# will-rowe/hulk

Measured on AMD Instinct MI355X. Metric: reads/sec (150bp, k=21, sketch=512), higher is better.
Workload: dtype u64

## Files before the change

### hulk_amd/csrc/hulk_minimizer.hip

```cpp
#include "hulk_minhash.h"

#include <type_traits>

#include <math.h>
#include <stdlib.h>
#include <algorithm>

namespace hulk {
namespace {

__device__ __forceinline__ uint8_t nt4_of(unsigned c) {
    unsigned u = c | 0x20u;
    if (c < 4) return (uint8_t)c;
    if (u == 'a') return 0;
    if (u == 'c') return 1;
    if (u == 'g') return 2;
    if (u == 't' || u == 'u') return 3;
    return 4;
}

template <bool MH>
__global__ __launch_bounds__(256) void k_minimizer_bin(const uint8_t *__restrict__ bases,
                                                       const uint64_t *__restrict__ offsets,
                                                       uint64_t n_reads, MinimizerParams P,
// ... 117 lines not shown
            if (lane == 0) vm[j0 >> 6] = vmask;
        }
        wave_sync();

        uint64_t carry_m = 0; bool carry_emit = false;
        for (int32_t j0 = 0; j0 < npos; j0 += 64) {
            const int32_t j = j0 + lane;
            const int32_t i = j + k - 1;
            const uint64_t vmask = vm[j0 >> 6];
            const bool emit = (j < npos) && ((vmask >> lane) & 1ull) && (i >= w - 1);
            uint64_t m = X_NONE;
            if (emit) {
                int32_t lo = j - (wwin - 1); if (lo < 0) lo = 0;
                for (int32_t p = lo; p <= j; p++) { const uint64_t x = Xs[p]; m = x < m ? x : m; }
            }
            uint64_t pm = __shfl_up(m, 1);
            int pe = __shfl_up((int)emit, 1);
            if (lane == 0) { pm = carry_m; pe = (int)carry_emit; }
            carry_m = __shfl(m, 63); carry_emit = __shfl((int)emit, 63) != 0;
            const bool start = emit && !(pe && pm == m);
            bool isnew = false;
            if (dbg & 8u) { sink += (uint32_t)m; } else
            if (dbg & 4u) { isnew = start; } else
            if (start) {
                uint32_t slot = ((uint32_t)(m >> 8) ^ (uint32_t)(m >> 37)) & tabmask;
                for (;;) {
                    const unsigned long long old =
                        atomicCAS((unsigned long long *)&tab[slot], (unsigned long long)TAB_EMPTY,
                                  (unsigned long long)m);
                    if (old == TAB_EMPTY) { isnew = true; break; }
                    if (old == m) break;
                    slot = (slot + 1) & tabmask;
                }
            }
            const uint64_t nb = __ballot(isnew);
            if (nb) {
                const uint32_t rank = __builtin_amdgcn_mbcnt_hi((uint32_t)(nb >> 32),
                                          __builtin_amdgcn_mbcnt_lo((uint32_t)nb, 0u));
                if (isnew) { q[qn + rank] = m; qs[qn + rank] = hslot; }
                qn += (uint32_t)__popcll(nb);
                wave_sync();
            }
            if (qn >= 64) {
                const uint64_t x = q[lane];
                const uint32_t xs = qs[lane];
                const uint64_t keep = (lane + 64u < qn) ? q[lane + 64] : 0;
                const uint32_t keeps = (lane + 64u < qn) ? qs[lane + 64] : 0;
                if (MH) mh_feed_wave(M, x, true, mh_min);
                const int32_t bin = (dbg & 2u) ? (int32_t)((uint32_t)(x >> 20) & 0xffffu) : jump_hash(x, P.num_bins);
                if (dbg & 1u) sink += (uint32_t)bin; else
                atomicAdd(&hist[(size_t)xs * (size_t)P.num_bins + bin], 1u);
                wave_sync();
                q[lane] = keep; qs[lane] = keeps;
                wave_sync();
                qn -= 64; nmin += 64;
            }
        }
        for (uint32_t s = lane; s < tabn; s += 64) tab[s] = TAB_EMPTY;
        wave_sync();
    }
    if (qn) {
        if (MH) mh_feed_wave(M, (uint32_t)lane < qn ? q[lane] : ~0ull, (uint32_t)lane < qn, mh_min);
        if ((uint32_t)lane < qn)
            atomicAdd(&hist[(size_t)qs[lane] * (size_t)P.num_bins + jump_hash(q[lane], P.num_bins)], 1u);
        nmin += qn;
    }
    if (MH) mh_finish_wave(M, mh_min);
    __shared__ unsigned long long blk_nmin[4];
    if (lane == 0) blk_nmin[wid] = nmin;
    __syncthreads();
    if (threadIdx.x == 0) {
        unsigned long long t = 0;
        for (int x = 0; x < nw; x++) t += blk_nmin[x];
        if (t) atomicAdd(&min_slots[blockIdx.x], t);
        if (MH && t) atomicAdd(&M.fed[blockIdx.x & (MH_FED_SLOTS - 1)], t);
    }
    if (dbg && sink == 0xdeadbeefu) hist[0] = sink;
}


#ifndef HULK_FAST_TAB
#define HULK_FAST_TAB 128
#endif
#ifndef HULK_FAST_PAD
#define HULK_FAST_PAD 0
#endif
constexpr int FAST_TAB = HULK_FAST_TAB;
constexpr int FAST_PAD = HULK_FAST_PAD;
constexpr int FAST_CAND = 64;
constexpr int FAST_NCH = 3, FAST_NCH_PAIR = 5;
constexpr int FAST_STREAM = (64 * FAST_NCH + 4) * 4;
constexpr int FAST_STREAM_PAIR = (64 * FAST_NCH_PAIR + 4) * 4;
constexpr uint32_t TAB_EMPTY32 = 0xFFFFFFFFu;
constexpr int FAST_TAB_BYTES = 16 * FAST_TAB * 4;
static_assert(FAST_TAB > FAST_CAND, "the set must keep more slots than a read can have candidates (finite probe loops)");
static_assert((FAST_TAB & (FAST_TAB - 1)) == 0 && FAST_TAB % 16 == 0, "slot masks and the per-lane clear");
static_assert(2 * FAST_CAND <= 0x7fffffff, "candidate indices must not reach TAB_EMPTY32");

__device__ __forceinline__ uint32_t dpp_row_shr1(uint32_t v) {
    return (uint32_t)__builtin_amdgcn_update_dpp(0, (int)v, 0x111, 0xf, 0xf, true);
}
__device__ __forceinline__ uint64_t dpp_row_shr1_u64(uint64_t v) {
    return (uint64_t)dpp_row_shr1((uint32_t)v) | ((uint64_t)dpp_row_shr1((uint32_t)(v >> 32)) << 32);
}

__device__ __forceinline__ uint64_t mul_u32_u64(uint32_t a, uint32_t b) {
    uint64_t d, carry;
    asm("v_mad_u64_u32 %0, %1, %2, %3, 0" : "=v"(d), "=s"(carry) : "v"(a), "s"(b));
    return d;
}
__device__ __forceinline__ uint32_t mad_u24(uint32_t a, uint32_t b, uint32_t c) {
    uint32_t d;
    asm("v_mad_u32_u24 %0, %1, %2, %3" : "=v"(d) : "v"(a), "s"(b), "v"(c));
    return d;
}
template <uint32_t B> __device__ __forceinline__ uint64_t mul_u32_u64_inl(uint32_t a) {
    static_assert(B <= 64, "inline constants are 0..64");
    uint64_t d, carry;
    asm("v_mad_u64_u32 %0, %1, %2, %3, 0" : "=v"(d), "=s"(carry) : "v"(a), "n"(B));
    return d;
}
template <uint32_t B> __device__ __forceinline__ uint32_t mad_u24_inl(uint32_t a, uint32_t c) {
    static_assert(B <= 64, "inline constants are 0..64");
    uint32_t d;
    asm("v_mad_u32_u24 %0, %1, %2, %3" : "=v"(d) : "v"(a), "n"(B), "v"(c));
    return d;
}
template <bool FM> __device__ __forceinline__ uint64_t hash64_fm(uint64_t key, uint64_t mask) {
    if (!FM) return hash64(key, mask);
    key = (~key + (key << 21)) & mask;
    key = key ^ key >> 24;
    {
        const uint64_t p = mul_u32_u64((uint32_t)key, 265u);
        const uint32_t hi = mad_u24((uint32_t)(key >> 32), 265u, (uint32_t)(p >> 32));
        key = (((uint64_t)hi << 32) | (uint32_t)p) & mask;
    }
    key = key ^ key >> 14;
    {
        const uint64_t p = mul_u32_u64((uint32_t)key, 21u);
        const uint32_t hi = mad_u24((uint32_t)(key >> 32), 21u, (uint32_t)(p >> 32));
        key = (((uint64_t)hi << 32) | (uint32_t)p) & mask;
    }
    key = key ^ key >> 28;
    key = (key + (key << 31)) & mask;
    return key;
}

__device__ __forceinline__ uint64_t mad_u32_u64_m1(uint32_t a, uint32_t b) {
    uint64_t d, carry;
    asm("v_mad_u64_u32 %0, %1, %2, %3, -1" : "=v"(d), "=s"(carry) : "v"(a), "s"(b));
    return d;
}
template <int KC> __device__ __forceinline__ uint64_t hash64_pack_kc(uint64_t key, uint32_t span) {
    static_assert(KC >= 17 && KC <= 27, "upper dword of the k-mer must have 2..22 bits");
    constexpr uint32_t HM = (1u << (2 * KC - 32)) - 1u;
    uint32_t lo = (uint32_t)key, hi = (uint32_t)(key >> 32);
    uint64_t p;
    p = mad_u32_u64_m1(lo, 0x1FFFFFu);
    hi = mad_u24(hi, 0x1FFFFFu, (uint32_t)(p >> 32)) & HM; lo = (uint32_t)p;
    lo ^= __builtin_amdgcn_alignbit(hi, lo, 24);
    p = mul_u32_u64(lo, 265u);
    hi = mad_u24(hi, 265u, (uint32_t)(p >> 32)) & HM; lo = (uint32_t)p;
    lo ^= __builtin_amdgcn_alignbit(hi, lo, 14);
    if (2 * KC - 32 > 14) hi ^= hi >> 14;
    p = mul_u32_u64_inl<21u>(lo);
    hi = mad_u24_inl<21u>(hi, (uint32_t)(p >> 32)) & HM; lo = (uint32_t)p;
    lo ^= __builtin_amdgcn_alignbit(hi, lo, 28);
    p = mul_u32_u64(lo, 0x80000001u);
    hi = ((uint32_t)(p >> 32) + hi) & HM; lo = (uint32_t)p;
    const uint32_t xh = __builtin_amdgcn_alignbit(hi, lo, 24), xl = (lo << 8) | span;
    return ((uint64_t)xh << 32) | xl;
}

__device__ constexpr uint64_t low_bits64(int n) { return n >= 64 ? ~0ull : n <= 0 ? 0ull : (1ull << (n & 63)) - 1; }

template <int C> __device__ __forceinline__ uint32_t sub_c_if(uint32_t x, uint32_t one) {
    static_assert(C >= 1 && C <= 16, "-C must be an inline constant");
    uint32_t d;
    asm("v_mad_i32_i24 %0, %1, %2, %3" : "=v"(d) : "v"(one), "n"(-C), "v"(x));
    return d;
}
__device__ __forceinline__ uint32_t sub_small_if(uint32_t x, uint32_t one, int c) {
    switch (c) {
    case 1: return sub_c_if<1>(x, one);   case 2: return sub_c_if<2>(x, one);   case 3: return sub_c_if<3>(x, one);
    case 4: return sub_c_if<4>(x, one);   case 5: return sub_c_if<5>(x, one);   case 6: return sub_c_if<6>(x, one);
    case 7: return sub_c_if<7>(x, one);   case 8: return sub_c_if<8>(x, one);   case 9: return sub_c_if<9>(x, one);
    case 10: return sub_c_if<10>(x, one); case 11: return sub_c_if<11>(x, one); case 12: return sub_c_if<12>(x, one);
    case 13: return sub_c_if<13>(x, one); case 14: return sub_c_if<14>(x, one); case 15: return sub_c_if<15>(x, one);
    default: return x - one * (uint32_t)c;
    }
}

template <bool FM> __device__ __forceinline__ uint64_t umin64(uint64_t a, uint64_t b) {
    if (FM) {
        double d;
        asm("v_min_f64 %0, %1, %2" : "=v"(d) : "v"(__longlong_as_double((long long)a)), "v"(__longlong_as_double((long long)b)));
        return (uint64_t)__double_as_longlong(d);
    }
    return a < b ? a : b;
}

template <int WM, bool DBG, bool WEQ, int KC> constexpr int fast_blocks_per_cu() {
    return (WM == 9 && !DBG && WEQ && (KC == 21 || KC == 31)) ? 5 : 4;
}
template <int WM, bool FM, bool DBG, bool WEQ, int KC, bool PAIR>
__global__ __launch_bounds__(256, (fast_blocks_per_cu<WM, DBG, WEQ, KC>())) void k_minimizer_fast(const uint8_t *__restrict__ bases,
                                                        const uint64_t *__restrict__ offsets,
                                                        uint64_t n_reads, MinimizerParams P,
                                                        MinimizerList ml, DevState *st,
                                                        unsigned long long *__restrict__ min_slots) {
    extern __shared__ __align__(16) unsigned char smem[];

    constexpr bool KEY5 = !FM && WEQ && KC == 31;
    constexpr bool FMM = FM || KEY5;
    constexpr uint64_t XN = FMM ? 0x7FF0000000000000ull : X_NONE;
    const int lane = lane_id(), wid = __builtin_amdgcn_readfirstlane((int)(threadIdx.x >> 6));
    const int grp = threadIdx.x >> 4, gl = threadIdx.x & 15, gsh = lane & 48;
    const int32_t k = KC ? KC : (int32_t)P.k, w = WEQ ? WM : (int32_t)P.w;
    const uint64_t mask = (1ull << (2 * k)) - 1;
    const uint64_t shift = (uint64_t)(2 * (k - 1));
    constexpr int NCH = PAIR ? FAST_NCH_PAIR : FAST_NCH;
    constexpr int STW = (PAIR ? FAST_STREAM_PAIR : FAST_STREAM) / 4;
    constexpr uint32_t STCAP = 16u * 64u * NCH;
    constexpr int RPI = PAIR ? 2 : 4;
    constexpr bool DX = KC != 0 && WEQ && 2 * (KC + WM - 1) <= 64;
    constexpr bool HP = FM && WEQ && KC >= 17 && KC <= 27;
#ifdef HULK_ANALYSIS_NO_NV
    constexpr bool NV = false;
#else
    constexpr bool NV = (DX && HP && 2 * (KC + WM) <= 64) || (!DX && WM <= 9);
#endif
    const int half = PAIR ? (grp & 1) : 0;
    const int sub = PAIR ? ((grp & 3) >> 1) : (grp & 3);
    const int32_t posoff = half ? 16 * w - (w - 1) : 0;
    uint32_t *tab = (uint32_t *)(smem + FAST_PAD) + (size_t)(PAIR ? (grp & ~1) : grp) * FAST_TAB;
    uint32_t *pk32 = (uint32_t *)(smem + FAST_PAD + FAST_TAB_BYTES) + grp * 20;
    uint32_t *pkn32 = (uint32_t *)(smem + FAST_PAD + FAST_TAB_BYTES + 16 * 20 * 4) + grp * 20;
    uint32_t *code32 = (uint32_t *)(smem + FAST_PAD + FAST_TAB_BYTES + 2 * 16 * 20 * 4) + (size_t)wid * (2 * STW);
    uint32_t *flag32 = code32 + STW;
    uint64_t *cs = (uint64_t *)(smem + FAST_PAD + FAST_TAB_BYTES + 2 * 16 * 20 * 4 + 4 * 2 * 4 * STW) + (size_t)grp * FAST_CAND;
    const uint64_t *csp = PAIR ? cs - (size_t)half * FAST_CAND : cs;
    {
        uint32_t *own = (uint32_t *)(smem + FAST_PAD) + (size_t)grp * FAST_TAB;
#pragma unroll
        for (int x = 0; x < FAST_TAB / 16; x++) own[gl + 16 * x] = TAB_EMPTY32;
    }
    __syncthreads();

    const uint64_t region = (uint64_t)blockIdx.x * 4 + (uint64_t)wid;
    const uint64_t wave_first = region * FAST_READS_PER_WAVE;
    uint64_t *xl = ml.x + region * ml.rcap;
    uint8_t *sl8 = ml.slot + region * ml.rcap;
    uint32_t wcount = 0;
    uint32_t dmask = 0;
    const uint32_t dbg = DBG ? P.debug : 0u;
    uint32_t sink = 0;
    if (blockIdx.x == 0 && threadIdx.x == 0 && n_reads)
        atomicAdd(&st->total_len, (unsigned long long)(offsets[n_reads] - offsets[0]));

    const uint32_t nrd = wave_first < n_reads ? (uint32_t)((n_reads - wave_first < FAST_READS_PER_WAVE) ? n_reads - wave_first : FAST_READS_PER_WAVE) : 0u;
    uint64_t myoff = 0;
    if ((uint32_t)lane <= nrd && nrd) myoff = offsets[wave_first + (uint32_t)lane];
    const uint32_t nrd_s = __builtin_amdgcn_readfirstlane(nrd);
    const uint64_t span_lo = (uint64_t)__builtin_amdgcn_readfirstlane((uint32_t)myoff) | (uint64_t)__builtin_amdgcn_readfirstlane((uint32_t)(myoff >> 32)) << 32;
    const uint64_t span_hi = (uint64_t)__builtin_amdgcn_readlane((uint32_t)myoff, nrd_s) | (uint64_t)__builtin_amdgcn_readlane((uint32_t)(myoff >> 32), nrd_s) << 32;
    const uintptr_t raw_a0 = ((uintptr_t)bases + span_lo) & ~(uintptr_t)15;
    const uintptr_t raw_end = (uintptr_t)bases + span_hi;
    const bool bulk = nrd && (raw_end - raw_a0) <= (uintptr_t)STCAP;
    const uint32_t delta = (uint32_t)(((uintptr_t)bases + span_lo) - raw_a0);
    bool anymark = false;
    if (bulk) {
        const uintptr_t lim = (uintptr_t)bases + P.bases_bytes;
        uint4 v[NCH]; bool whole[NCH];
        const bool first_ok = raw_a0 < lim;
#pragma unroll
        for (int x = 0; x < NCH; x++) {
            const uintptr_t a = raw_a0 + 16u * (uint32_t)(lane + 64 * x);
            whole[x] = a < raw_end + 16 && a < lim;
            v[x] = first_ok ? *(const uint4 *)(whole[x] ? a : raw_a0) : make_uint4(0, 0, 0, 0);
        }
        const uint32_t endoff = (uint32_t)(raw_end - raw_a0);
        bool marked = false;
#pragma unroll
        for (int x = 0; x < NCH; x++) {
            const uint32_t d[4] = {v[x].x, v[x].y, v[x].z, v[x].w};
            uint32_t pack = 0, fpack = 0, bad = 0;
#pragma unroll
            for (int y = 0; y < 4; y++) {
                const uint32_t up = d[y] & 0xDFDFDFDFu;
                const uint32_t e = up >> 1;
                const uint32_t c = (e ^ (e >> 1)) & 0x03030303u;
                bad |= __builtin_amdgcn_perm(0u, 0x54474341u, c) ^ up;
                pack |= ((c * 0x01041040u) >> 24) << (8 * y);
            }
            if (!whole[x]) { pack = 0; bad = 0; }
            if (bad != 0) {
                const int32_t c0 = 16 * (lane + 64 * x);
                const int32_t lo = (int32_t)delta - c0, hi = (int32_t)endoff - c0;
#pragma unroll
                for (int y = 0; y < 4; y++) {
                    const uint32_t by = d[y], up = by & 0xDFDFDFDFu, e = up >> 1, c = (e ^ (e >> 1)) & 0x03030303u;
                    const int nl = lo - 4 * y, nh = hi - 4 * y;
                    const uint32_t ml = nl >= 4 ? ~0u : nl <= 0 ? 0u : (1u << (8 * nl)) - 1u;
                    const uint32_t mh = nh >= 4 ? ~0u : nh <= 0 ? 0u : (1u << (8 * nh)) - 1u;
                    const uint32_t mm = (__builtin_amdgcn_perm(0u, 0x54474341u, c) ^ up) & mh & ~ml;
                    const uint32_t nz = (((mm & 0x7F7F7F7Fu) + 0x7F7F7F7Fu) | mm) & 0x80808080u;
                    uint32_t hard4 = nz >> 7, soft4 = 0;
                    if (NV) {
                        const uint32_t tU = up ^ 0x55555555u, t3 = by & 0xFCFCFCFCu;
                        const uint32_t isU = ~(((tU & 0x7F7F7F7Fu) + 0x7F7F7F7Fu) | tU | 0x7F7F7F7Fu);
                        const uint32_t is03 = ~(((t3 & 0x7F7F7F7Fu) + 0x7F7F7F7Fu) | t3 | 0x7F7F7F7Fu);
                        hard4 = (nz & is03) >> 7;
                        soft4 = (nz & ~isU & ~is03) >> 7;
                    }
                    const uint32_t b4 = soft4 | (hard4 << 1);
                    const uint32_t fl = (b4 & 3u) | ((b4 >> 6) & 12u) | ((b4 >> 12) & 48u) | ((b4 >> 18) & 192u);
                    fpack |= fl << (8 * y);
                }
                pack &= ~((fpack & 0x55555555u) * 3u);
            }
            code32[lane + 64 * x] = pack;
            flag32[lane + 64 * x] = fpack;
            marked = marked || fpack != 0;
        }
        if (lane < 4) { code32[64 * NCH + lane] = 0u; flag32[64 * NCH + lane] = 0u; }
        anymark = __ballot(marked) != 0ull;
    }
    wave_sync();
// ... 60 lines not shown
        if (BULK) {
            cw = code32; fw = flag32;
            cb = a32 + (uint32_t)ap0; cb = cb < STCAP ? cb : STCAP;
            if (anymark) {
                Xn = win64(fw, ap0 ? cb - 1u : cb);
                if (ap0 == 0) Xn <<= 2;
                uint64_t seen;
                if (DX) {
                    constexpr int NBW = KC + WM - 1;
                    Xn &= low_bits64(2 * (NBW + 1));
                    seen = Xn;
                } else {
                    const uint32_t at = cb + (uint32_t)k;
                    nn = win32(fw, at < STCAP ? at : STCAP);
                    seen = Xn | nn;
                }
                const bool counts = act && !defer && p0 < nposg;
                sawN = counts && (seen & 0xAAAAAAAAAAAAAAAAull) != 0;
                softN = NV && counts && (seen & 0x5555555555555555ull) != 0;
                Xn &= 0x5555555555555555ull;
            }
        } else if (act && !defer) {
            const int32_t p = 16 * gl;
            uint32_t pack = 0, npack = 0;
            if (p < Lg) {
                const uint32_t ro = a32 + (uint32_t)posoff + (uint32_t)p;
                unsigned sh;
                uint32_t d[5];
                {
                    const uintptr_t addr = raw_a0 + ro;
                    const uintptr_t al = addr & ~(uintptr_t)3, end = (uintptr_t)bases + P.bases_bytes;
                    sh = (unsigned)(addr & 3) * 8;
#pragma unroll
                    for (int x = 0; x < 5; x++) d[x] = (al + 4 * x < end) ? *(const uint32_t *)(al + 4 * x) : 0u;
                }
                uint32_t bad = 0;
#pragma unroll
                for (int x = 0; x < 4; x++) {
                    const uint32_t by = __builtin_amdgcn_alignbit(d[x + 1], d[x], sh);
                    const uint32_t up = by & 0xDFDFDFDFu;
                    const uint32_t e = up >> 1;
                    const uint32_t c = (e ^ (e >> 1)) & 0x03030303u;
                    bad |= __builtin_amdgcn_perm(0u, 0x54474341u, c) ^ up;
                    pack |= ((c * 0x01041040u) >> 24) << (8 * x);
                }
                const bool lastread = Lg - p < 16 && lastwave && idx + 1 == nrd;
                if (bad != 0 || lastread) {
                    const int nv = lastread ? (int)(Lg - p) : 16;
                    uint32_t hard = 0;
#pragma unroll
                    for (int x = 0; x < 4; x++) {
                        const uint32_t by = __builtin_amdgcn_alignbit(d[x + 1], d[x], sh);
                        const uint32_t up = by & 0xDFDFDFDFu, e = up >> 1, c = (e ^ (e >> 1)) & 0x03030303u;
                        const int nb = nv - 4 * x;
                        const uint32_t m = nb >= 4 ? ~0u : nb <= 0 ? 0u : (1u << (8 * nb)) - 1u;
                        const uint32_t mm = (__builtin_amdgcn_perm(0u, 0x54474341u, c) ^ up) & m;
                        if (NV) {
                            const uint32_t nz = (((mm & 0x7F7F7F7Fu) + 0x7F7F7F7Fu) | mm) & 0x80808080u;
                            const uint32_t tU = up ^ 0x55555555u, t3 = by & 0xFCFCFCFCu;
                            const uint32_t isU = ~(((tU & 0x7F7F7F7Fu) + 0x7F7F7F7Fu) | tU | 0x7F7F7F7Fu);
                            const uint32_t is03 = ~(((t3 & 0x7F7F7F7Fu) + 0x7F7F7F7Fu) | t3 | 0x7F7F7F7Fu);
                            hard |= nz & is03;
                            const uint32_t b4 = (nz & ~isU & ~is03) >> 7;
                            const uint32_t fl = (b4 & 1u) | ((b4 >> 6) & 4u) | ((b4 >> 12) & 16u) | ((b4 >> 18) & 64u);
                            npack |= fl << (8 * x);
                        } else hard |= mm;
                    }
                    sawN = hard != 0;
                    softN = NV && npack != 0;
                    if (NV) pack &= ~(npack * 3u);
                }
            }
            pk32[gl] = pack;
            if (glq < 4) pk32[16 + gl] = 0;
            if (NV) { pkn32[gl] = npack; if (glq < 4) pkn32[16 + gl] = 0; }
        }
        const bool voting = !BULK || anymark;
        if (voting) {
            const uint32_t gN = PAIR ? (uint32_t)(__ballot(sawN) >> (lane & 32)) : (uint32_t)(__ballot(sawN) >> gsh) & 0xffffu;
            if (gN) defer = true;
        }
        const bool waveN = NV && voting && __ballot(softN && !defer) != 0ull;
        if (!BULK) wave_sync();
        if (dbg & 32u) { sink += cw[gl]; wave_sync(); return; }

        const bool mine = act && !defer && p0 < nposg;
        uint32_t validbits = 0;
        uint64_t X[WM];
#pragma unroll
        for (int t = 0; t < WM; t++) if (!WEQ || t >= w) X[t] = XN;
        {
            if (mine) validbits = (1u << (nposg - p0 < w ? nposg - p0 : w)) - 1u;
            const int32_t span0 = ap0 + k - 1 - w + 2;
            uint64_t f = 0, r = 0;
            uint32_t nb = 0;
            uint64_t Bb = 0, Cl = 0;
            uint64_t Hb = 0;
            if (NV && waveN && !BULK) {
                const uint32_t bo = 2u * (uint32_t)p0, nbo = p0 > 0 ? bo - 2u : 0u, d = nbo >> 5, o = nbo & 31u;
                const uint64_t lo = (uint64_t)pkn32[d] | ((uint64_t)pkn32[d + 1] << 32);
                Xn = o ? (lo >> o) | ((uint64_t)pkn32[d + 2] << (64 - o)) : lo;
                if (p0 == 0) {
                    Xn <<= 2;
                    if (PAIR && half) {
                        const uint32_t q = (uint32_t)(posoff - 1);
                        Xn |= (uint64_t)(((pkn32 - 20)[q >> 4] >> (2u * (q & 15u))) & 1u);
                    }
                }
            }
            if (DX) {
                constexpr int NBW = DX ? KC + WM - 1 : 1;
                uint64_t Wl = win64(cw, cb);
                Wl &= low_bits64(2 * NBW);
                const uint64_t rv = __brevll(Wl) >> (64 - 2 * NBW);
                Bb = ((rv >> 1) & 0x5555555555555555ull) | ((rv & 0x5555555555555555ull) << 1);
                Cl = ~Wl;
            } else {
                {
                    uint64_t W = win64(cw, cb);
                    W &= mask;
                    r = (~W) & mask;
                    if (NV && waveN) {
                        const uint64_t X0 = Xn & low_bits64(2 * k + 2);
                        W |= (X0 >> 4) & (mask >> 2);
                        r |= X0 & ((mask << 1) | 1ull);
                    }
                    const uint64_t rev = __brevll(W) >> (64 - 2 * k);
                    f = ((rev >> 1) & 0x5555555555555555ull) | ((rev & 0x5555555555555555ull) << 1);
                }
                {
                    uint32_t at = cb + (uint32_t)k;
                    if (BULK) at = at < STCAP ? at : STCAP;
                    nb = win32(cw, at);
                    if (NV && waveN && !BULK) nn = win32(fw, at);
                }
            }
            if (NV && DX && waveN) {
                constexpr int NBW = DX ? KC + WM - 1 : 1;
                Xn &= low_bits64(2 * (NBW + 1));
                const uint64_t Fn = (Xn >> 4) & low_bits64(2 * (NBW - 1));
                const uint64_t rv = __brevll(Fn) >> (64 - 2 * NBW);
                Hb = ((rv >> 1) & 0x5555555555555555ull) | ((rv & 0x5555555555555555ull) << 1);
            }
            uint32_t ap0_now = (uint32_t)ap0;
            if (KC != 0 && WEQ) asm volatile("" : "+v"(ap0_now));
            const bool first_block = ap0_now == 0u;
            const uint32_t fb1 = first_block ? 1u : 0u;
            auto phaseA = [&](auto nvx_tag) {
            constexpr bool NVX = decltype(nvx_tag)::value;
#pragma unroll
            for (int t = 0; t < WM; t++) {
                if (DX) {
                    constexpr int HB = 2 * KC - 32;
                    const int sf = 2 * (WM - 1 - t), sr = 2 * t;
                    const uint32_t bl = (uint32_t)Bb, cl = (uint32_t)Cl;
                    uint32_t bh = (uint32_t)(Bb >> 32), ch = (uint32_t)(Cl >> 32);
                    asm("" : "+v"(bh), "+v"(ch));
                    uint32_t fl = sf ? __builtin_amdgcn_alignbit(bh, bl, sf) : bl, fh = __builtin_amdgcn_ubfe(bh, sf, HB);
                    uint32_t rl = sr ? __builtin_amdgcn_alignbit(ch, cl, sr) : cl, rh = __builtin_amdgcn_ubfe(ch, sr, HB);
                    if (NVX) {
                        const uint32_t hl = (uint32_t)Hb, xl = (uint32_t)Xn;
                        uint32_t hh = (uint32_t)(Hb >> 32), xh = (uint32_t)(Xn >> 32);
                        asm("" : "+v"(hh), "+v"(xh));
                        fl |= (sf ? __builtin_amdgcn_alignbit(hh, hl, sf) : hl) & ~3u; fh |= __builtin_amdgcn_ubfe(hh, sf, HB);
                        rl |= sr ? __builtin_amdgcn_alignbit(xh, xl, sr) : xl; rh |= __builtin_amdgcn_ubfe(xh, sr, HB + 1);
                    }
                    f = ((uint64_t)fh << 32) | fl;
                    r = ((uint64_t)rh << 32) | rl;
                } else if (t) {
                    uint64_t c = nb & 3u; nb >>= 2;
                    if (NVX) { c |= (uint64_t)(nn & 1u) << 2; nn >>= 2; }
                    f = (f << 2 | c) & mask;
                    r = (r >> 2) | ((3ull ^ c) << shift);
                }
                if (t < w) {
                    const uint64_t canon = (NVX && k >= 31) ? (f < r ? f : r) : umin64<true>(f, r);
                    int32_t span;
                    if (KC != 0 && WEQ) span = k;
                    else { span = span0 + t; if (span >= k) span = k; }
                    uint64_t x;
                    if (HP && !(dbg & 16u)) x = hash64_pack_kc<HP ? KC : 21>(canon, (uint32_t)span);
                    else if (KEY5) x = (hash64(canon, mask) & 0x00FFFFFFFFFFFFFFull) << 5 | (uint64_t)(uint32_t)span;
                    else x = ((dbg & 16u) ? canon * 0x9E3779B97F4A7C15ull : hash64_fm<FM>(canon, mask)) << 8 | (uint64_t)(int64_t)span;
                    if (KC != 0 && WEQ && t < w - 1) x = (x & 0xffffffff00000000ull) | sub_small_if((uint32_t)x, fb1, w - 1 - t);
                    if ((NVX || !(k & 1)) && f == r) { x = XN; validbits &= ~(1u << t); }
                    X[t] = x;
                }
            }
            };
            if (NV && waveN) phaseA(std::true_type{}); else phaseA(std::false_type{});
        }
        if (dbg & 8u) {
#pragma unroll
            for (int t = 0; t < WM; t++) sink += (uint32_t)X[t];
            wave_sync();
            return;
        }

        uint32_t startbits = 0;
        {
            uint64_t hp[WM];
            {
                uint64_t h = XN;
#pragma unroll
                for (int t = WM - 1; t >= 0; t--) {
                    if (t < w) h = umin64<FMM>(X[t], h);
                    hp[t] = h;
                }
            }
            const uint64_t whole = dpp_row_shr1_u64(hp[0]);
            const uint64_t xnfix = glq == 0 ? XN : 0ull;
#pragma unroll
            for (int t = 0; t < WM - 1; t++) {
                const uint64_t v = dpp_row_shr1_u64(hp[t + 1]);
                hp[t] = FMM ? (v | (xnfix & 0xffffffff00000000ull)) : (v | xnfix);
            }
            hp[WM - 1] = XN;
            const uint32_t pv = dpp_row_shr1(validbits);
            uint32_t eqbits = 0;
            uint64_t g = XN, pm = whole;
#pragma unroll
            for (int t = 0; t < WM; t++) {
                g = umin64<FMM>(X[t], g);
                const uint64_t hpt = (t + 1 < w) ? hp[t] : XN;
                const uint64_t m = umin64<FMM>(hpt, g);
                if (t < w) { eqbits |= (m == pm) ? (1u << t) : 0u; pm = m; }
                X[t] = m;
            }
            uint32_t emitbits = validbits;
            {
                const int32_t t1 = (w - 1) - (k - 1) - ap0;
                if (t1 > 0) emitbits &= ~((1u << t1) - 1u);
                if (PAIR && halfq) { const int32_t t2 = (w - 1) - p0; if (t2 > 0) emitbits &= ~((1u << t2) - 1u); }
            }
            const uint32_t pe0 = (glq > 0 && ((pv >> (w - 1)) & 1u) && (ap0 - 1 + k - 1 >= w - 1) && !(halfq && p0 - 1 < w - 1)) ? 1u : 0u;
            startbits = emitbits & ~(((emitbits << 1) | pe0) & eqbits);
        }
        uint32_t total;
        {
            const uint32_t cnt = (uint32_t)__popc(startbits);
            uint32_t incl = cnt;
            incl += dpp_row_shr1(incl);
            incl += (uint32_t)__builtin_amdgcn_update_dpp(0, (int)incl, 0x112, 0xf, 0xf, true);
            incl += (uint32_t)__builtin_amdgcn_update_dpp(0, (int)incl, 0x114, 0xf, 0xf, true);
            incl += (uint32_t)__builtin_amdgcn_update_dpp(0, (int)incl, 0x118, 0xf, 0xf, true);
            total = (uint32_t)__shfl((int)incl, (lane & 48) | 15);
            bool ovf = total > (uint32_t)FAST_CAND;
            if (PAIR) ovf = ((uint32_t)(__ballot(ovf) >> (lane & 32))) != 0u;
            if (ovf) { defer = true; total = 0; }
            else {
                uint32_t at = incl - cnt;
#pragma unroll
                for (int t = 0; t < WM; t++)
                    if ((startbits >> t) & 1u) cs[at++] = X[t];
            }
        }
        {
            const uint64_t dbal = __ballot(act && defer && glq == 0 && halfq == 0);
            if (PAIR) dmask |= ((uint32_t)(dbal & 1u) | ((uint32_t)(dbal >> 32) & 1u) << 1) << (RPI * it);
            else dmask |= ((uint32_t)(dbal & 1u) | ((uint32_t)(dbal >> 16) & 1u) << 1 | ((uint32_t)(dbal >> 32) & 1u) << 2 |
                           ((uint32_t)(dbal >> 48) & 1u) << 3) << (RPI * it);
            if (act && defer) act = false;
        }
        wave_sync();

        uint32_t myslot[FAST_CAND / 16];
        uint32_t newmask = 0;
        constexpr uint32_t TABM = (PAIR ? 2 * FAST_TAB : FAST_TAB) - 1;
#pragma unroll
        for (int pr = 0; pr < FAST_CAND / 32; pr++) {
            const uint32_t c0 = (uint32_t)gl + 32u * (uint32_t)pr, c1 = c0 + 16u;
            myslot[2 * pr] = 0; myslot[2 * pr + 1] = 0;
            if (!__any((int)(c0 < total))) break;
            const bool a0 = c0 < total, a1 = c1 < total;
            uint64_t x0 = 0, x1 = 0;
            if (a0) x0 = cs[c0];
            if (a1) x1 = cs[c1];
            const uint64_t r0 = x0, r1 = x1;
            if (KEY5) { x0 = (x0 & ~31ull) << 3 | (x0 & 31ull); x1 = (x1 & ~31ull) << 3 | (x1 & 31ull); }
            uint32_t sl0 = ((uint32_t)(x0 >> 8) ^ (uint32_t)(x0 >> 37)) & TABM, sl1 = ((uint32_t)(x1 >> 8) ^ (uint32_t)(x1 >> 37)) & TABM;
            const uint32_t i0 = (PAIR ? (uint32_t)half * FAST_CAND : 0u) + c0, i1 = i0 + 16u;
            uint32_t o0 = TAB_EMPTY32, o1 = TAB_EMPTY32;
            if (!(dbg & 4u)) {
                if (a0) o0 = atomicCAS(&tab[sl0], TAB_EMPTY32, i0);
                if (a1) o1 = atomicCAS(&tab[sl1], TAB_EMPTY32, i1);
                while (a0 && o0 != TAB_EMPTY32 && csp[o0] != r0) {
                    sl0 = (sl0 + 1) & TABM;
                    o0 = atomicCAS(&tab[sl0], TAB_EMPTY32, i0);
                }
                while (a1 && o1 != TAB_EMPTY32 && csp[o1] != r1) {
                    sl1 = (sl1 + 1) & TABM;
                    o1 = atomicCAS(&tab[sl1], TAB_EMPTY32, i1);
                }
            }
            const bool new0 = a0 && o0 == TAB_EMPTY32, new1 = a1 && o1 == TAB_EMPTY32;
            myslot[2 * pr] = sl0; myslot[2 * pr + 1] = sl1;
            const uint64_t nb0 = __ballot(new0), nb1 = __ballot(new1);
            if (nb0 | nb1) {
                const uint32_t n0 = (uint32_t)__popcll(nb0);
                if (new0) {
                    const uint32_t rank = __builtin_amdgcn_mbcnt_hi((uint32_t)(nb0 >> 32), __builtin_amdgcn_mbcnt_lo((uint32_t)nb0, 0u));
                    newmask |= 1u << (2 * pr);
                    if (dbg & 1u) sink += (uint32_t)x0; else { xl[wcount + rank] = x0; sl8[wcount + rank] = (uint8_t)hslot; }
                }
                if (new1) {
                    const uint32_t rank = n0 + __builtin_amdgcn_mbcnt_hi((uint32_t)(nb1 >> 32), __builtin_amdgcn_mbcnt_lo((uint32_t)nb1, 0u));
                    newmask |= 2u << (2 * pr);
                    if (dbg & 1u) sink += (uint32_t)x1; else { xl[wcount + rank] = x1; sl8[wcount + rank] = (uint8_t)hslot; }
                }
                wcount += n0 + (uint32_t)__popcll(nb1);
            }
        }
        wave_sync();
#pragma unroll
        for (int rnd = 0; rnd < FAST_CAND / 16; rnd++)
            if ((newmask >> rnd) & 1u) tab[myslot[rnd]] = TAB_EMPTY32;
        wave_sync();
    };
    if (bulk) {
        for (int it = 0; it < FAST_READS_PER_WAVE / RPI && (uint32_t)(RPI * it) < nrd; it++) trip(std::true_type{}, it);
    } else if (!wide) {
        for (int it = 0; it < FAST_READS_PER_WAVE / RPI && (uint32_t)(RPI * it) < nrd; it++) trip(std::false_type{}, it);
    } else dmask = (1u << nrd_s) - 1u;
    if (lane == 0 && wave_first < n_reads) { ml.cnt[region] = wcount; ml.dmask[region] = dmask; }
    if (dbg && sink == 0xdeadbeefu) xl[0] = sink;
    __shared__ unsigned long long blk_nmin[4];
    if (lane == 0) blk_nmin[wid] = wcount;
    __syncthreads();
    if (threadIdx.x == 0) {
        const unsigned long long t = blk_nmin[0] + blk_nmin[1] + blk_nmin[2] + blk_nmin[3];
        if (t) atomicAdd(&min_slots[blockIdx.x & (MIN_SLOTS - 1)], t);
    }
}

#ifndef HULK_LONG_PPT
#define HULK_LONG_PPT 8
#endif
constexpr int LONG_PPT = HULK_LONG_PPT;
__global__ __launch_bounds__(256) void k_long_hash(const uint8_t *__restrict__ bases, const LongSeqDesc *__restrict__ desc,
                                                   MinimizerParams P, uint64_t *__restrict__ Xs_all,
                                                   uint8_t *__restrict__ valid_all) {
    __shared__ uint8_t lut[256];
    for (int t = threadIdx.x; t < 256; t += blockDim.x) lut[t] = nt4_of((unsigned)t);
    __syncthreads();
    const LongSeqDesc d = desc[blockIdx.y];
    const uint8_t *seq = bases + d.seq_off;
    uint64_t *Xs = Xs_all + d.xs_off;
    uint8_t *valid = valid_all + d.xs_off;
    const int64_t k = (int64_t)P.k, w = (int64_t)P.w;
    const uint64_t mask = (1ull << (2 * k)) - 1, shift = (uint64_t)(2 * (k - 1));
    const uint64_t npos = d.L - (uint64_t)k + 1;
    for (uint64_t j0 = ((uint64_t)blockIdx.x * blockDim.x + threadIdx.x) * LONG_PPT; j0 < npos;
         j0 += (uint64_t)gridDim.x * blockDim.x * LONG_PPT) {
        const uint64_t jend = j0 + LONG_PPT < npos ? j0 + LONG_PPT : npos;
        uint64_t f = 0, r = 0;
        for (int64_t p = j0 > 0 ? (int64_t)j0 - 1 : 0; p < (int64_t)jend + k - 1; p++) {
            const uint64_t c = lut[seq[p]];
            f = (f << 2 | c) & mask;
            r = (r >> 2) | ((3ull ^ c) << shift);
            const int64_t j = p - (k - 1);
            if (j < (int64_t)j0) continue;
            uint64_t X = X_NONE; uint8_t ok = 0;
            if (f != r) {
                const uint64_t canon = f > r ? r : f;
                int64_t span = p - w + 2;
                if (span >= k) span = k;
                X = hash64(canon, mask) << 8 | (uint64_t)(int64_t)(int32_t)span;
                ok = 1;
            }
            Xs[j] = X; valid[j] = ok;
        }
    }
}

__global__ __launch_bounds__(256) void k_long_emit(const LongSeqDesc *__restrict__ desc, const uint64_t *__restrict__ Xs_all,
                                                   const uint8_t *__restrict__ valid_all, MinimizerParams P,
                                                   uint64_t *__restrict__ table_all, uint32_t *__restrict__ hists,
                                                   unsigned long long *__restrict__ min_slots) {
    __shared__ unsigned red[4];
    constexpr unsigned QCAP = 2048;
    __shared__ uint64_t q[QCAP];
    __shared__ unsigned qn;
    if (threadIdx.x == 0) qn = 0;
    __syncthreads();
    const LongSeqDesc d = desc[blockIdx.y];
    const uint64_t *Xs = Xs_all + d.xs_off;
    const uint8_t *valid = valid_all + d.xs_off;
    uint64_t *table = table_all + d.tab_off;
    const uint64_t table_mask = d.tab_mask;
    uint32_t *hist = hists + (size_t)d.hslot * (size_t)P.num_bins;
    const int64_t k = (int64_t)P.k, w = (int64_t)P.w;
    const uint64_t wwin = (uint64_t)(w > 0 ? w : 1);
    const uint64_t npos = d.L - (uint64_t)k + 1;
    unsigned fresh = 0;
    for (uint64_t j0 = ((uint64_t)blockIdx.x * blockDim.x + threadIdx.x) * LONG_PPT; j0 < npos;
         j0 += (uint64_t)gridDim.x * blockDim.x * LONG_PPT) {
        const uint64_t jend = j0 + LONG_PPT < npos ? j0 + LONG_PPT : npos;
        uint64_t m = X_NONE, mprev = X_NONE;
// ... 130 lines not shown
                        const unsigned long long old = atomicCAS((unsigned long long *)&table[slot], (unsigned long long)TAB_EMPTY,
                                                                 (unsigned long long)m);
                        if (old == TAB_EMPTY) {
                            const unsigned at = atomicAdd(&qn, 1u);
                            if (at < QCAP) q[at] = m; else atomicAdd(&hist[jump_hash(m, P.num_bins)], 1u);
                            fresh++;
                            break;
                        }
                        if (old == m) break;
                        slot = (slot + 1) & table_mask;
                    }
                }
                prev_emit = emit; mprev = m;
            }
        }
        __syncthreads();
        {
#ifdef HULK_EXPERIMENTS
            if ((P.debug & LONG_TILE_LAG) && tid >= 64) {
                for (int i = 0; i < 10; i++) __builtin_amdgcn_s_sleep(127);
                __atomic_signal_fence(__ATOMIC_SEQ_CST);
            }
#endif
            const unsigned nq = qn < QCAP ? qn : QCAP;
            for (unsigned i = tid; i < nq; i += 256) atomicAdd(&hist[jump_hash(q[i], P.num_bins)], 1u);
        }
    }
    for (int off = 32; off; off >>= 1) fresh += __shfl_xor(fresh, off);
    if (lane_id() == 0) red[tid >> 6] = fresh;
    __syncthreads();
    if (tid == 0) {
        const unsigned t = red[0] + red[1] + red[2] + red[3];
        if (t) atomicAdd(&min_slots[(blockIdx.x + 131u * blockIdx.y) & (MIN_SLOTS - 1)], (unsigned long long)t);
    }
}

__global__ void k_fill_u64(uint64_t *p, uint64_t n, uint64_t v) {
    for (uint64_t i = (uint64_t)blockIdx.x * blockDim.x + threadIdx.x; i < n; i += (uint64_t)gridDim.x * blockDim.x) p[i] = v;
}

}

size_t minimizer_lds_per_wave(uint32_t xcap, uint32_t tab_size) {
    size_t words = (size_t)xcap + (xcap + 63) / 64 + tab_size + 128 + 64;
    size_t pk = ((size_t)xcap + 32 + 3) / 4 + 16;
    pk = (pk + 7) & ~(size_t)7;
    return words * 8 + 2 * pk;
}

size_t minimizer_lds_per_block(uint32_t xcap, uint32_t tab_size, int waves) {
    return 256 + (size_t)waves * minimizer_lds_per_wave(xcap, tab_size);
}

hipError_t launch_minimizer_bin(hipStream_t s, const uint8_t *d_bases, const uint64_t *d_offsets,
                                uint64_t n_reads, MinimizerParams P, int block_threads,
                                uint32_t *d_hist, DevState *d_state, unsigned long long *d_min_slots,
                                const uint32_t *d_read_list, const uint32_t *d_read_list_count,
                                uint32_t list_blocks, const MinHashState *mh) {
    if (n_reads == 0) return hipSuccess;
    const int waves = block_threads / 64;
    P.lds_per_wave = (uint32_t)minimizer_lds_per_wave(P.xcap, P.tab_size);
    const size_t lds = minimizer_lds_per_block(P.xcap, P.tab_size, waves);
    uint64_t blocks = (n_reads + (uint64_t)waves * 4 - 1) / ((uint64_t)waves * 4);
    if (blocks > MIN_SLOTS) blocks = MIN_SLOTS;
    if (blocks < 1) blocks = 1;
    if (d_read_list) blocks = list_blocks;
    const bool feed = mh && mh->mode;
    if (lds > 64 * 1024) {
        hipError_t e = hipFuncSetAttribute(feed ? (const void *)k_minimizer_bin<true> : (const void *)k_minimizer_bin<false>,
                                           hipFuncAttributeMaxDynamicSharedMemorySize, (int)lds);
        if (e != hipSuccess) return e;
    }
    prof_mark(s, "k_minimizer_bin");
    if (feed)
        hipLaunchKernelGGL(k_minimizer_bin<true>, dim3((unsigned)blocks), dim3(block_threads), lds, s, d_bases,
                           d_offsets, n_reads, P, d_hist, d_state, d_min_slots, d_read_list, d_read_list_count, *mh);
    else
        hipLaunchKernelGGL(k_minimizer_bin<false>, dim3((unsigned)blocks), dim3(block_threads), lds, s, d_bases,
                           d_offsets, n_reads, P, d_hist, d_state, d_min_slots, d_read_list, d_read_list_count, MinHashState{});
    return hipGetLastError();
}

constexpr size_t fast_lds_bytes(bool pair) {
    return FAST_PAD + (size_t)FAST_TAB_BYTES + 2 * 16 * 20 * 4 + 4 * 2 * (size_t)(pair ? FAST_STREAM_PAIR : FAST_STREAM) + 16 * (size_t)FAST_CAND * 8;
}
constexpr size_t FAST_LDS_GRANULE = 1280, FAST_LDS_STATIC = 32, CU_LDS_BYTES = 160 * 1024;
constexpr size_t fast_lds_alloc(bool pair) { return (fast_lds_bytes(pair) + FAST_LDS_STATIC + FAST_LDS_GRANULE - 1) / FAST_LDS_GRANULE * FAST_LDS_GRANULE; }
#if HULK_FAST_PAD == 0 && HULK_FAST_TAB == 128
static_assert(fast_blocks_per_cu<9, false, true, 21>() == 5 && fast_blocks_per_cu<9, false, true, 31>() == 5, "the default instances are built for 5 workgroups per CU");
static_assert(6 * fast_lds_alloc(false) <= CU_LDS_BYTES, "k_minimizer_fast: the LDS no longer admits 6 workgroups per CU (its registers are budgeted for 5)");
static_assert(5 * fast_lds_alloc(true) <= CU_LDS_BYTES, "k_minimizer_fast (PAIR): the LDS no longer admits the 5 workgroups per CU its registers are budgeted for");
#endif
size_t minimizer_fast_lds(uint32_t, bool pair) { return fast_lds_bytes(pair); }

hipError_t launch_minimizer_fast(hipStream_t s, const uint8_t *d_bases, const uint64_t *d_offsets,
                                 uint64_t n_reads, MinimizerParams P, const MinimizerList &ml,
                                 DevState *d_state, unsigned long long *d_min_slots) {
    if (n_reads == 0) return hipSuccess;
    const bool pair = P.pair != 0;
    size_t lds = minimizer_fast_lds(P.w, pair);
    {
        static const char *e = HULK_EXP_ENV("HULK_K1_LDS_TOTAL");
        static const size_t want = e ? (size_t)atol(e) : 0;
        if (want > lds) {
            static bool once = false;
            if (!once && want > 65536) { once = true; (void)hipFuncSetAttribute((const void *)k_minimizer_fast<9, false, false, true, 31, false>, hipFuncAttributeMaxDynamicSharedMemorySize, (int)want); }
            lds = want;
        }
    }
    const uint64_t blocks = (n_reads + 4 * FAST_READS_PER_WAVE - 1) / (4 * FAST_READS_PER_WAVE);
    const dim3 g((unsigned)blocks), b(256);
    static const bool no_fmin = HULK_EXP_ENV("HULK_NO_FMIN") != nullptr;
    const bool fm = P.k <= 27 && !no_fmin;
    prof_mark(s, "k_minimizer_fast");
#define HULK_LAUNCH_FAST3(WM, FMv, DBGv, WEQv, KCv, PAIRv)                                                           \
    hipLaunchKernelGGL((k_minimizer_fast<WM, FMv, DBGv, WEQv, KCv, PAIRv>), g, b, lds, s, d_bases, d_offsets, n_reads, \
                       P, ml, d_state, d_min_slots)
#define HULK_LAUNCH_FAST2(WM, FMv, DBGv, WEQv, KCv)                                                                  \
    do { if (pair) HULK_LAUNCH_FAST3(WM, FMv, DBGv, WEQv, KCv, true); else HULK_LAUNCH_FAST3(WM, FMv, DBGv, WEQv, KCv, false); } while (0)
#define HULK_LAUNCH_FAST(WM)                                                                                         \
    do {                                                                                                             \
        const bool weq = P.w == WM;                                                                                  \
        if (P.debug) HULK_LAUNCH_FAST2(WM, false, true, false, 0);                                                   \
        else if (fm && weq && P.k == 21) HULK_LAUNCH_FAST2(WM, true, false, true, 21);    \
        else if (!fm && weq && P.k == 31) HULK_LAUNCH_FAST2(WM, false, false, true, 31);           \
        else if (fm && weq) HULK_LAUNCH_FAST2(WM, true, false, true, 0);                                             \
        else if (fm) HULK_LAUNCH_FAST2(WM, true, false, false, 0);                                                   \
        else if (weq) HULK_LAUNCH_FAST2(WM, false, false, true, 0);                                                  \
        else HULK_LAUNCH_FAST2(WM, false, false, false, 0);                                                          \
    } while (0)
    if (P.w <= 4) HULK_LAUNCH_FAST(4);
    else if (P.w <= 9) HULK_LAUNCH_FAST(9);
    else HULK_LAUNCH_FAST(16);
#undef HULK_LAUNCH_FAST3
#undef HULK_LAUNCH_FAST2
#undef HULK_LAUNCH_FAST
    return hipGetLastError();
}

uint32_t minimizer_list_rcap(uint32_t w, bool pair) {
    static const uint32_t pad = [] { const char *e = HULK_EXP_ENV("HULK_RCAP_PAD"); return e ? (uint32_t)atol(e) : 64u; }();
    const uint32_t by_pos = FAST_READS_PER_WAVE * (pair ? 2u * 16u * w - (w - 1u) : 16u * w);
    const uint32_t by_cand = FAST_READS_PER_WAVE * (uint32_t)FAST_CAND * (pair ? 2u : 1u);
    return by_pos < by_cand + pad ? by_pos : by_cand + pad;
}

hipError_t launch_long_group(hipStream_t s, const uint8_t *d_bases, const LongSeqDesc *d_desc, uint32_t n_seqs,
                             uint64_t max_npos, MinimizerParams P, uint64_t *d_xs, uint8_t *d_valid, uint64_t *d_table,
                             uint64_t table_total, uint32_t *d_hists, unsigned long long *d_min_slots) {
    prof_mark(s, "k_fill_u64");
    hipLaunchKernelGGL(k_fill_u64, dim3(4096), dim3(256), 0, s, d_table, table_total, TAB_EMPTY);
    if (d_xs && d_valid) {
        uint64_t bx = (max_npos + 256 * LONG_PPT - 1) / (256 * LONG_PPT);
        const uint64_t cap = std::max<uint64_t>(1, 131072 / n_seqs);
        if (bx > cap) bx = cap;
        if (bx > 8192) bx = 8192;
        prof_mark(s, "k_long_hash");
        hipLaunchKernelGGL(k_long_hash, dim3((unsigned)bx, n_seqs), dim3(256), 0, s, d_bases, d_desc, P, d_xs, d_valid);
        prof_mark(s, "k_long_emit");
        hipLaunchKernelGGL(k_long_emit, dim3((unsigned)bx, n_seqs), dim3(256), 0, s, d_desc, d_xs, d_valid, P, d_table,
                           d_hists, d_min_slots);
        return hipGetLastError();
    }
    const uint64_t H = (((uint64_t)(P.w ? P.w : 1) + 7) & ~7ull), TP = (uint64_t)LONG_TILE - H;
    uint64_t bx = (max_npos + TP - 1) / TP;
    const uint64_t cap = std::max<uint64_t>(1, 262144 / n_seqs);
    if (bx > cap) bx = cap;
    if (bx > 65535) bx = 65535;
    if (const char *e = HULK_EXP_ENV("HULK_LONG_TILE_GRID")) { const long n = atol(e); if (n > 0 && bx > (uint64_t)n) bx = (uint64_t)n; }
    if (HULK_EXP_ENV("HULK_LONG_TILE_LAG")) P.debug |= LONG_TILE_LAG;
    prof_mark(s, "k_long_tile");
    hipLaunchKernelGGL(k_long_tile, dim3((unsigned)bx, n_seqs), dim3(256), 0, s, d_bases, d_desc, P, d_table, d_hists, d_min_slots);
    return hipGetLastError();
}

}
```

Before: 2.164 billion.

## Shrink single-read LDS footprint to fit seven workgroups per CU on headline path

Drops the per-group candidate cap from 64 to 48 for single-end reads. It also removes the separate pk32/pkn32 staging buffers by aliasing them into the per-wave code/flag streams, so the single-end LDS allocation shrinks. The headline instance (w=9, k=21, single-end) gets launch bounds of 7 workgroups per CU, and the bit offset is taken from a pinned register cb. The aim is higher occupancy. The risks are register spills under the tighter budget and more reads overflowing the smaller candidate set and being deferred to a slower path.

```diff
diff --git a/hulk_amd/csrc/hulk_minimizer.hip b/hulk_amd/csrc/hulk_minimizer.hip
--- a/hulk_amd/csrc/hulk_minimizer.hip
+++ b/hulk_amd/csrc/hulk_minimizer.hip
@@ -223,20 +223,26 @@
 #ifndef HULK_FAST_TAB
 #define HULK_FAST_TAB 128
 #endif
+#ifndef HULK_FAST_TAB_SINGLE
+#define HULK_FAST_TAB_SINGLE 128
+#endif
 #ifndef HULK_FAST_PAD
 #define HULK_FAST_PAD 0
 #endif
-constexpr int FAST_TAB = HULK_FAST_TAB;
 constexpr int FAST_PAD = HULK_FAST_PAD;
-constexpr int FAST_CAND = 64;
+constexpr int fast_tab(bool pair) { return pair ? HULK_FAST_TAB : HULK_FAST_TAB_SINGLE; }
+constexpr int fast_cand(bool pair) { return pair ? 64 : 48; }
 constexpr int FAST_NCH = 3, FAST_NCH_PAIR = 5;
 constexpr int FAST_STREAM = (64 * FAST_NCH + 4) * 4;
 constexpr int FAST_STREAM_PAIR = (64 * FAST_NCH_PAIR + 4) * 4;
 constexpr uint32_t TAB_EMPTY32 = 0xFFFFFFFFu;
-constexpr int FAST_TAB_BYTES = 16 * FAST_TAB * 4;
-static_assert(FAST_TAB > FAST_CAND, "the set must keep more slots than a read can have candidates (finite probe loops)");
-static_assert((FAST_TAB & (FAST_TAB - 1)) == 0 && FAST_TAB % 16 == 0, "slot masks and the per-lane clear");
-static_assert(2 * FAST_CAND <= 0x7fffffff, "candidate indices must not reach TAB_EMPTY32");
+constexpr int fast_tab_bytes(bool pair) { return 16 * fast_tab(pair) * 4; }
+static_assert(fast_tab(false) > fast_cand(false) && fast_tab(true) > fast_cand(true),
+              "the set must keep more slots than a read can have candidates (finite probe loops)");
+static_assert((fast_tab(false) & (fast_tab(false) - 1)) == 0 && fast_tab(false) % 16 == 0 &&
+              (fast_tab(true) & (fast_tab(true) - 1)) == 0 && fast_tab(true) % 16 == 0, "slot masks and the per-lane clear");
+static_assert(fast_cand(false) % 16 == 0 && fast_cand(true) % 16 == 0, "candidates are taken 16 per round (one per lane of a group)");
+static_assert(2 * fast_cand(true) <= 0x7fffffff, "candidate indices must not reach TAB_EMPTY32");
 
 __device__ __forceinline__ uint32_t dpp_row_shr1(uint32_t v) {
     return (uint32_t)__builtin_amdgcn_update_dpp(0, (int)v, 0x111, 0xf, 0xf, true);
@@ -341,11 +347,15 @@
     return a < b ? a : b;
 }
 
-template <int WM, bool DBG, bool WEQ, int KC> constexpr int fast_blocks_per_cu() {
+#ifndef HULK_FAST_HEADLINE_BLOCKS
+#define HULK_FAST_HEADLINE_BLOCKS 7
+#endif
+template <int WM, bool DBG, bool WEQ, int KC, bool PAIR> constexpr int fast_blocks_per_cu() {
+    if (WM == 9 && !DBG && WEQ && KC == 21 && !PAIR) return HULK_FAST_HEADLINE_BLOCKS;
     return (WM == 9 && !DBG && WEQ && (KC == 21 || KC == 31)) ? 5 : 4;
 }
 template <int WM, bool FM, bool DBG, bool WEQ, int KC, bool PAIR>
-__global__ __launch_bounds__(256, (fast_blocks_per_cu<WM, DBG, WEQ, KC>())) void k_minimizer_fast(const uint8_t *__restrict__ bases,
+__global__ __launch_bounds__(256, (fast_blocks_per_cu<WM, DBG, WEQ, KC, PAIR>())) void k_minimizer_fast(const uint8_t *__restrict__ bases,
                                                         const uint64_t *__restrict__ offsets,
                                                         uint64_t n_reads, MinimizerParams P,
                                                         MinimizerList ml, DevState *st,
@@ -371,20 +381,22 @@
 #else
     constexpr bool NV = (DX && HP && 2 * (KC + WM) <= 64) || (!DX && WM <= 9);
 #endif
+    constexpr int TABN = fast_tab(PAIR), CAND = fast_cand(PAIR), TAB_BYTES = fast_tab_bytes(PAIR);
     const int half = PAIR ? (grp & 1) : 0;
     const int sub = PAIR ? ((grp & 3) >> 1) : (grp & 3);
     const int32_t posoff = half ? 16 * w - (w - 1) : 0;
-    uint32_t *tab = (uint32_t *)(smem + FAST_PAD) + (size_t)(PAIR ? (grp & ~1) : grp) * FAST_TAB;
-    uint32_t *pk32 = (uint32_t *)(smem + FAST_PAD + FAST_TAB_BYTES) + grp * 20;
-    uint32_t *pkn32 = (uint32_t *)(smem + FAST_PAD + FAST_TAB_BYTES + 16 * 20 * 4) + grp * 20;
-    uint32_t *code32 = (uint32_t *)(smem + FAST_PAD + FAST_TAB_BYTES + 2 * 16 * 20 * 4) + (size_t)wid * (2 * STW);
+    uint32_t *tab = (uint32_t *)(smem + FAST_PAD) + (size_t)(PAIR ? (grp & ~1) : grp) * TABN;
+    uint32_t *code32 = (uint32_t *)(smem + FAST_PAD + TAB_BYTES) + (size_t)wid * (2 * STW);
     uint32_t *flag32 = code32 + STW;
-    uint64_t *cs = (uint64_t *)(smem + FAST_PAD + FAST_TAB_BYTES + 2 * 16 * 20 * 4 + 4 * 2 * 4 * STW) + (size_t)grp * FAST_CAND;
-    const uint64_t *csp = PAIR ? cs - (size_t)half * FAST_CAND : cs;
+    uint32_t *pk32 = code32 + (grp & 3) * 20;
+    uint32_t *pkn32 = flag32 + (grp & 3) * 20;
+    static_assert(4 * 20 <= STW, "the per-trip staging of a wave's four groups fits in each of its streams");
+    uint64_t *cs = (uint64_t *)(smem + FAST_PAD + TAB_BYTES + 4 * 2 * 4 * STW) + (size_t)grp * CAND;
+    const uint64_t *csp = PAIR ? cs - (size_t)half * CAND : cs;
     {
-        uint32_t *own = (uint32_t *)(smem + FAST_PAD) + (size_t)grp * FAST_TAB;
-#pragma unroll
-        for (int x = 0; x < FAST_TAB / 16; x++) own[gl + 16 * x] = TAB_EMPTY32;
+        uint32_t *own = (uint32_t *)(smem + FAST_PAD) + (size_t)grp * TABN;
+#pragma unroll
+        for (int x = 0; x < TABN / 16; x++) own[gl + 16 * x] = TAB_EMPTY32;
     }
     __syncthreads();
 
@@ -611,6 +623,7 @@
         }
         const bool waveN = NV && voting && __ballot(softN && !defer) != 0ull;
         if (!BULK) wave_sync();
+        if (!BULK && KC != 0 && WEQ) asm volatile("" : "+v"(cb));
         if (dbg & 32u) { sink += cw[gl]; wave_sync(); return; }
 
         const bool mine = act && !defer && p0 < nposg;
@@ -626,7 +639,7 @@
             uint64_t Bb = 0, Cl = 0;
             uint64_t Hb = 0;
             if (NV && waveN && !BULK) {
-                const uint32_t bo = 2u * (uint32_t)p0, nbo = p0 > 0 ? bo - 2u : 0u, d = nbo >> 5, o = nbo & 31u;
+                const uint32_t bo = 2u * cb, nbo = p0 > 0 ? bo - 2u : 0u, d = nbo >> 5, o = nbo & 31u;
                 const uint64_t lo = (uint64_t)pkn32[d] | ((uint64_t)pkn32[d + 1] << 32);
                 Xn = o ? (lo >> o) | ((uint64_t)pkn32[d + 2] << (64 - o)) : lo;
                 if (p0 == 0) {
@@ -774,7 +787,7 @@
             incl += (uint32_t)__builtin_amdgcn_update_dpp(0, (int)incl, 0x114, 0xf, 0xf, true);
             incl += (uint32_t)__builtin_amdgcn_update_dpp(0, (int)incl, 0x118, 0xf, 0xf, true);
             total = (uint32_t)__shfl((int)incl, (lane & 48) | 15);
-            bool ovf = total > (uint32_t)FAST_CAND;
+            bool ovf = total > (uint32_t)CAND;
             if (PAIR) ovf = ((uint32_t)(__ballot(ovf) >> (lane & 32))) != 0u;
             if (ovf) { defer = true; total = 0; }
             else {
@@ -793,22 +806,24 @@
         }
         wave_sync();
 
-        uint32_t myslot[FAST_CAND / 16];
+        constexpr int NRND = CAND / 16;
+        uint32_t myslot[NRND];
         uint32_t newmask = 0;
-        constexpr uint32_t TABM = (PAIR ? 2 * FAST_TAB : FAST_TAB) - 1;
-#pragma unroll
-        for (int pr = 0; pr < FAST_CAND / 32; pr++) {
+        constexpr uint32_t TABM = (PAIR ? 2 * TABN : TABN) - 1;
+#pragma unroll
+        for (int pr = 0; pr < (NRND + 1) / 2; pr++) {
+            const bool two = 2 * pr + 1 < NRND;
             const uint32_t c0 = (uint32_t)gl + 32u * (uint32_t)pr, c1 = c0 + 16u;
-            myslot[2 * pr] = 0; myslot[2 * pr + 1] = 0;
+            myslot[2 * pr] = 0; if (two) myslot[2 * pr + 1] = 0;
             if (!__any((int)(c0 < total))) break;
-            const bool a0 = c0 < total, a1 = c1 < total;
+            const bool a0 = c0 < total, a1 = two && c1 < total;
             uint64_t x0 = 0, x1 = 0;
             if (a0) x0 = cs[c0];
             if (a1) x1 = cs[c1];
             const uint64_t r0 = x0, r1 = x1;
             if (KEY5) { x0 = (x0 & ~31ull) << 3 | (x0 & 31ull); x1 = (x1 & ~31ull) << 3 | (x1 & 31ull); }
             uint32_t sl0 = ((uint32_t)(x0 >> 8) ^ (uint32_t)(x0 >> 37)) & TABM, sl1 = ((uint32_t)(x1 >> 8) ^ (uint32_t)(x1 >> 37)) & TABM;
-            const uint32_t i0 = (PAIR ? (uint32_t)half * FAST_CAND : 0u) + c0, i1 = i0 + 16u;
+            const uint32_t i0 = (PAIR ? (uint32_t)half * CAND : 0u) + c0, i1 = i0 + 16u;
             uint32_t o0 = TAB_EMPTY32, o1 = TAB_EMPTY32;
             if (!(dbg & 4u)) {
                 if (a0) o0 = atomicCAS(&tab[sl0], TAB_EMPTY32, i0);
@@ -823,7 +838,7 @@
                 }
             }
             const bool new0 = a0 && o0 == TAB_EMPTY32, new1 = a1 && o1 == TAB_EMPTY32;
-            myslot[2 * pr] = sl0; myslot[2 * pr + 1] = sl1;
+            myslot[2 * pr] = sl0; if (two) myslot[2 * pr + 1] = sl1;
             const uint64_t nb0 = __ballot(new0), nb1 = __ballot(new1);
             if (nb0 | nb1) {
                 const uint32_t n0 = (uint32_t)__popcll(nb0);
@@ -842,7 +857,7 @@
         }
         wave_sync();
 #pragma unroll
-        for (int rnd = 0; rnd < FAST_CAND / 16; rnd++)
+        for (int rnd = 0; rnd < NRND; rnd++)
             if ((newmask >> rnd) & 1u) tab[myslot[rnd]] = TAB_EMPTY32;
         wave_sync();
     };
@@ -1139,14 +1154,18 @@
 }
 
 constexpr size_t fast_lds_bytes(bool pair) {
-    return FAST_PAD + (size_t)FAST_TAB_BYTES + 2 * 16 * 20 * 4 + 4 * 2 * (size_t)(pair ? FAST_STREAM_PAIR : FAST_STREAM) + 16 * (size_t)FAST_CAND * 8;
+    return FAST_PAD + (size_t)fast_tab_bytes(pair) + 4 * 2 * (size_t)(pair ? FAST_STREAM_PAIR : FAST_STREAM) + 16 * (size_t)fast_cand(pair) * 8;
 }
 constexpr size_t FAST_LDS_GRANULE = 1280, FAST_LDS_STATIC = 32, CU_LDS_BYTES = 160 * 1024;
 constexpr size_t fast_lds_alloc(bool pair) { return (fast_lds_bytes(pair) + FAST_LDS_STATIC + FAST_LDS_GRANULE - 1) / FAST_LDS_GRANULE * FAST_LDS_GRANULE; }
-#if HULK_FAST_PAD == 0 && HULK_FAST_TAB == 128
-static_assert(fast_blocks_per_cu<9, false, true, 21>() == 5 && fast_blocks_per_cu<9, false, true, 31>() == 5, "the default instances are built for 5 workgroups per CU");
-static_assert(6 * fast_lds_alloc(false) <= CU_LDS_BYTES, "k_minimizer_fast: the LDS no longer admits 6 workgroups per CU (its registers are budgeted for 5)");
-static_assert(5 * fast_lds_alloc(true) <= CU_LDS_BYTES, "k_minimizer_fast (PAIR): the LDS no longer admits the 5 workgroups per CU its registers are budgeted for");
+#if HULK_FAST_PAD == 0 && HULK_FAST_TAB == 128 && HULK_FAST_TAB_SINGLE == 128 && HULK_FAST_HEADLINE_BLOCKS == 7
+static_assert(fast_blocks_per_cu<9, false, true, 21, false>() == 7, "the headline instance is built for 7 workgroups per CU");
+static_assert(fast_blocks_per_cu<9, false, true, 21, true>() == 5 && fast_blocks_per_cu<9, false, true, 31, false>() == 5 &&
+              fast_blocks_per_cu<9, false, true, 31, true>() == 5, "the other default instances are built for 5 workgroups per CU");
+static_assert(fast_lds_alloc(false) == 21760 && 7 * fast_lds_alloc(false) <= CU_LDS_BYTES,
+              "k_minimizer_fast: the LDS no longer admits the 7 workgroups per CU the headline's registers are budgeted for");
+static_assert(fast_lds_alloc(true) == 26880 && 6 * fast_lds_alloc(true) <= CU_LDS_BYTES,
+              "k_minimizer_fast (PAIR): the LDS no longer admits 6 workgroups per CU (its registers are budgeted for 5)");
 #endif
 size_t minimizer_fast_lds(uint32_t, bool pair) { return fast_lds_bytes(pair); }
 
@@ -1198,7 +1217,7 @@
 uint32_t minimizer_list_rcap(uint32_t w, bool pair) {
     static const uint32_t pad = [] { const char *e = HULK_EXP_ENV("HULK_RCAP_PAD"); return e ? (uint32_t)atol(e) : 64u; }();
     const uint32_t by_pos = FAST_READS_PER_WAVE * (pair ? 2u * 16u * w - (w - 1u) : 16u * w);
-    const uint32_t by_cand = FAST_READS_PER_WAVE * (uint32_t)FAST_CAND * (pair ? 2u : 1u);
+    const uint32_t by_cand = FAST_READS_PER_WAVE * (uint32_t)fast_cand(true) * (pair ? 2u : 1u);
     return by_pos < by_cand + pad ? by_pos : by_cand + pad;
 }
 
```

Result: no change. 2.179 billion, median of 6 (+0.7%).
